# hrnr/map-merge

Hardware: NVIDIA B200
Metric: pairwise_registrations_per_sec (higher is better)
Workload: dtype f32

## Files before the change

map-merge_b200/csrc/exact_math.h:

```cpp
#pragma once
#include <math.h>
#include <stdint.h>
#include <string.h>

#if defined(__CUDACC__)
#define MM_HD __host__ __device__ __forceinline__
#else
#define MM_HD inline
#endif

namespace mm3d {
namespace em {

MM_HD double bits_to_double(uint64_t u)
{
  double d;
  memcpy(&d, &u, sizeof(d));
  return d;
}

MM_HD float bits_to_float(uint32_t u)
{
  float f;
  memcpy(&f, &u, sizeof(f));
  return f;
}

MM_HD float expf_(float x)
{
  if (x != x) return x;
  if (x < -104.0f) return 0.0f;
  if (x > 88.72f) return INFINITY;
  const float n = rintf(x * 1.44269504088896341f);
  float r = x - n * 0.693359375f;
  r = r - n * -2.12194440e-4f;
  float p = 1.9875691500e-4f;
  p = p * r + 1.3981999507e-3f;
  p = p * r + 8.3334519073e-3f;
  p = p * r + 4.1665795894e-2f;
  p = p * r + 1.6666665459e-1f;
  p = p * r + 5.0000001201e-1f;
  const float y = (p * (r * r) + r) + 1.0f;
  int ni = (int)n;
  const int h = ni / 2;
  const float s1 = bits_to_float((uint32_t)(127 + h) << 23);
  const float s2 = bits_to_float((uint32_t)(127 + (ni - h)) << 23);
  return (y * s1) * s2;
}

MM_HD float atanf_pos_(float x, float* lo)
{
  float y0, y0lo;
  if (x > 2.414213562373095f) {
    y0 = 1.57079637050628662109375f;
    y0lo = -4.37113900018624283e-8f;
    x = -(1.0f / x);
  } else if (x > 0.4142135623730950f) {
    y0 = 0.785398185253143310546875f;
    y0lo = -2.18556950009312142e-8f;
    x = (x - 1.0f) / (x + 1.0f);
  } else {
    y0 = 0.0f;
    y0lo = 0.0f;
  }
  const float z = x * x;
  float p = 8.05374449538e-2f;
  p = p * z - 1.38776856032e-1f;
  p = p * z + 1.99777106478e-1f;
  p = p * z - 3.33329491539e-1f;
  const float corr = p * z * x + y0lo;
  const float hi = y0 + x;
  *lo = ((y0 - hi) + x) + corr;
  return hi;
}

MM_HD float atan2f_(float y, float x)
{
  if (x != x || y != y) return x + y;
  const float ax = fabsf(x), ay = fabsf(y);
  float hi = 0.0f, lo = 0.0f;
  if (!(ax == 0.0f && ay == 0.0f)) hi = atanf_pos_(ay / ax, &lo);
  float a;
  if (signbit(x)) {
    const float d = 3.1415927410125732421875f - hi;
    a = d + (-8.74227800037248566e-8f - lo);
  } else {
    a = hi + lo;
  }
  return signbit(y) ? -a : a;
}

MM_HD double cos_small_(double t)
{
  const double t2 = t * t;
  double s = 1.0 / 6402373705728000.0;
  s = 1.0 / 20922789888000.0 - t2 * s;
  s = 1.0 / 87178291200.0 - t2 * s;
  s = 1.0 / 479001600.0 - t2 * s;
  s = 1.0 / 3628800.0 - t2 * s;
  s = 1.0 / 40320.0 - t2 * s;
  s = 1.0 / 720.0 - t2 * s;
  s = 1.0 / 24.0 - t2 * s;
  s = 0.5 - t2 * s;
  return 1.0 - t2 * s;
}

MM_HD double sin_small_(double t)
{
  const double t2 = t * t;
  double s = 1.0 / 121645100408832000.0;
  s = 1.0 / 355687428096000.0 - t2 * s;
  s = 1.0 / 1307674368000.0 - t2 * s;
  s = 1.0 / 6227020800.0 - t2 * s;
  s = 1.0 / 39916800.0 - t2 * s;
  s = 1.0 / 362880.0 - t2 * s;
  s = 1.0 / 5040.0 - t2 * s;
  s = 1.0 / 120.0 - t2 * s;
  s = 1.0 / 6.0 - t2 * s;
  return t * (1.0 - t2 * s);
}

MM_HD float cosf_small_(float t) { return (float)cos_small_((double)t); }
MM_HD float sinf_small_(float t) { return (float)sin_small_((double)t); }

template <typename T>
MM_HD T sqrt_(T v);
template <>
MM_HD float sqrt_<float>(float v) { return sqrtf(v); }
template <>
MM_HD double sqrt_<double>(double v) { return sqrt(v); }

template <typename T>
MM_HD T det3(const T* m)
{
  return m[0] * (m[4] * m[8] - m[5] * m[7]) - m[1] * (m[3] * m[8] - m[5] * m[6]) +
         m[2] * (m[3] * m[7] - m[4] * m[6]);
}

template <typename T>
MM_HD void svd3(const T* A, T* U, T* s, T* V)
{
  T a[9];
  for (int i = 0; i < 9; ++i) {
    a[i] = A[i];
    V[i] = T(0);
  }
  V[0] = V[4] = V[8] = T(1);
  const T eps = sizeof(T) == 4 ? T(1.1920929e-7) : T(2.220446049250313e-16);
  for (int sweep = 0; sweep < 30; ++sweep) {
    bool rotated = false;
    for (int p = 0; p < 2; ++p) {
      for (int q = p + 1; q < 3; ++q) {
        T alpha = T(0), beta = T(0), gamma = T(0);
        for (int i = 0; i < 3; ++i) {
          alpha += a[i * 3 + p] * a[i * 3 + p];
          beta += a[i * 3 + q] * a[i * 3 + q];
          gamma += a[i * 3 + p] * a[i * 3 + q];
        }
        if (gamma == T(0)) continue;
        if (fabs(gamma) <= eps * sqrt_<T>(alpha * beta)) continue;
        rotated = true;
        const T zeta = (beta - alpha) / (T(2) * gamma);
        const T t = (zeta >= T(0) ? T(1) : T(-1)) / (fabs(zeta) + sqrt_<T>(T(1) + zeta * zeta));
        const T c = T(1) / sqrt_<T>(T(1) + t * t);
        const T sn = c * t;
        for (int i = 0; i < 3; ++i) {
          const T ap = a[i * 3 + p], aq = a[i * 3 + q];
          a[i * 3 + p] = c * ap - sn * aq;
          a[i * 3 + q] = sn * ap + c * aq;
          const T vp = V[i * 3 + p], vq = V[i * 3 + q];
          V[i * 3 + p] = c * vp - sn * vq;
          V[i * 3 + q] = sn * vp + c * vq;
        }
      }
    }
    if (!rotated) break;
  }
  T n[3];
  for (int j = 0; j < 3; ++j)
    n[j] = sqrt_<T>(a[j] * a[j] + a[3 + j] * a[3 + j] + a[6 + j] * a[6 + j]);
  int ord[3] = {0, 1, 2};
  for (int i = 0; i < 2; ++i)
    for (int j = i + 1; j < 3; ++j)
      if (n[ord[j]] > n[ord[i]]) {
        int tmp = ord[i];
        ord[i] = ord[j];
        ord[j] = tmp;
      }
  T Vs[9], As[9];
  for (int j = 0; j < 3; ++j) {
    s[j] = n[ord[j]];
    for (int i = 0; i < 3; ++i) {
      Vs[i * 3 + j] = V[i * 3 + ord[j]];
      As[i * 3 + j] = a[i * 3 + ord[j]];
    }
  }
  for (int i = 0; i < 9; ++i) V[i] = Vs[i];
  const T tiny = s[0] * eps * T(8);
  int rank = 0;
  for (int j = 0; j < 3; ++j)
// ... 154 lines not shown
  const float* v;
  float l;
  if (l1 >= l2 && l1 >= l3) {
    v = v1;
    l = l1;
  } else if (l2 >= l1 && l2 >= l3) {
    v = v2;
    l = l2;
  } else {
    v = v3;
    l = l3;
  }
  const float inv = sqrtf(l);
  vec[0] = v[0] / inv;
  vec[1] = v[1] / inv;
  vec[2] = v[2] / inv;
}

MM_HD void eig3_sym_d(const double* a_in, double* val, double* vec)
{
  double a[9];
  for (int i = 0; i < 9; ++i) {
    a[i] = a_in[i];
    vec[i] = 0.0;
  }
  vec[0] = vec[4] = vec[8] = 1.0;
  for (int sweep = 0; sweep < 50; ++sweep) {
    const double off = a[1] * a[1] + a[2] * a[2] + a[5] * a[5];
    const double diag = a[0] * a[0] + a[4] * a[4] + a[8] * a[8];
    if (off <= 1e-32 * diag || off == 0.0) break;
    for (int p = 0; p < 2; ++p)
      for (int q = p + 1; q < 3; ++q) {
        const double apq = a[p * 3 + q];
        if (apq == 0.0) continue;
        const double theta = (a[q * 3 + q] - a[p * 3 + p]) / (2.0 * apq);
        const double t = (theta >= 0.0 ? 1.0 : -1.0) / (fabs(theta) + sqrt(theta * theta + 1.0));
        const double c = 1.0 / sqrt(t * t + 1.0), sn = t * c;
        for (int k = 0; k < 3; ++k) {
          const double akp = a[k * 3 + p], akq = a[k * 3 + q];
          a[k * 3 + p] = c * akp - sn * akq;
          a[k * 3 + q] = sn * akp + c * akq;
        }
        for (int k = 0; k < 3; ++k) {
          const double apk = a[p * 3 + k], aqk = a[q * 3 + k];
          a[p * 3 + k] = c * apk - sn * aqk;
          a[q * 3 + k] = sn * apk + c * aqk;
        }
        for (int k = 0; k < 3; ++k) {
          const double vkp = vec[k * 3 + p], vkq = vec[k * 3 + q];
          vec[k * 3 + p] = c * vkp - sn * vkq;
          vec[k * 3 + q] = sn * vkp + c * vkq;
        }
      }
  }
  val[0] = a[0];
  val[1] = a[4];
  val[2] = a[8];
  for (int i = 0; i < 2; ++i)
    for (int j = i + 1; j < 3; ++j)
      if (val[j] < val[i]) {
        const double tv = val[i];
        val[i] = val[j];
        val[j] = tv;
        for (int k = 0; k < 3; ++k) {
          const double tt = vec[k * 3 + i];
          vec[k * 3 + i] = vec[k * 3 + j];
          vec[k * 3 + j] = tt;
        }
      }
}

MM_HD double atan01_d_(double z)
{
  z = z / (1.0 + sqrt(1.0 + z * z));
  z = z / (1.0 + sqrt(1.0 + z * z));
  const double z2 = z * z;
  double s = 1.0 / 23.0;
  s = 1.0 / 21.0 - z2 * s;
  s = 1.0 / 19.0 - z2 * s;
  s = 1.0 / 17.0 - z2 * s;
  s = 1.0 / 15.0 - z2 * s;
  s = 1.0 / 13.0 - z2 * s;
  s = 1.0 / 11.0 - z2 * s;
  s = 1.0 / 9.0 - z2 * s;
  s = 1.0 / 7.0 - z2 * s;
  s = 1.0 / 5.0 - z2 * s;
  s = 1.0 / 3.0 - z2 * s;
  s = 1.0 - z2 * s;
  return 4.0 * (z * s);
}
MM_HD double atan2_d_(double y, double x)
{
  const double kPi = 3.14159265358979323846;
  if (x != x || y != y) return x + y;
  const double ax = fabs(x), ay = fabs(y);
  double a;
  if (ax == 0.0 && ay == 0.0) a = 0.0;
  else if (ay <= ax) a = atan01_d_(ay / ax);
  else a = 0.5 * kPi - atan01_d_(ax / ay);
  if (signbit(x)) a = kPi - a;
  return signbit(y) ? -a : a;
}
MM_HD double acos_d_(double c)
{
  return atan2_d_(sqrt((1.0 - c) * (1.0 + c)), c);
}

MM_HD float dist2_3(float ax, float ay, float az, float bx, float by, float bz)
{
  const float dx = ax - bx, dy = ay - by, dz = az - bz;
  float r = dx * dx;
  r += dy * dy;
  r += dz * dz;
  return r;
}

MM_HD void transform_point(const float* m, float x, float y, float z, float* ox, float* oy, float* oz)
{
  *ox = ((m[0] * x + m[1] * y) + m[2] * z) + m[3];
  *oy = ((m[4] * x + m[5] * y) + m[6] * z) + m[7];
  *oz = ((m[8] * x + m[9] * y) + m[10] * z) + m[11];
}

#define MM3D_FIX1_SCALE 4294967296.0
#define MM3D_FIX2_SCALE 16777216.0
#define MM3D_FIXD_SCALE 68719476736.0
MM_HD long long to_fix(double v, double scale)
{
#if defined(__CUDA_ARCH__)
  return __double2ll_rn(v * scale);
#else
  return (long long)rint(v * scale);
#endif
}

MM_HD long long to_fix32_pos(float v)
{
  unsigned int b;
#if defined(__CUDA_ARCH__)
  b = __float_as_uint(v);
#else
  memcpy(&b, &v, 4);
#endif
  const int e = (int)((b >> 23) & 0xffu);
  const unsigned long long m = (unsigned long long)(b & 0x7fffffu) | (e ? 0x800000ull : 0ull);
  const int sh = (e ? e : 1) - 118;
  if (sh >= 0) return (long long)(m << sh);
  const int s = -sh;
  if (s > 25) return 0;
  const unsigned long long r = m >> s, rem = m & ((1ull << s) - 1ull), half = 1ull << (s - 1);
  return (long long)(r + ((rem > half || (rem == half && (r & 1ull))) ? 1ull : 0ull));
}

}
}
```

map-merge_b200/csrc/features.cu:

```cuda
#include <algorithm>
#include <cmath>
#include <limits>

#include "mm3d_internal.cuh"
#include "pair_features.cuh"

namespace mm3d {

namespace {

constexpr int FB = 128;

static int radius_voxels(double radius, float leaf) { return (int)std::ceil(radius / (double)leaf) + 1; }

static int max_n(const std::vector<CloudView>& in)
{
  int mx = 0;
  for (const CloudView& v : in) mx = std::max(mx, v.n);
  return mx;
}

static std::vector<Seg> make_segs(const std::vector<int>& ns, int* total)
{
  std::vector<Seg> segs(ns.size());
  int off = 0;
  for (size_t m = 0; m < ns.size(); ++m) {
    segs[m].off = off;
    segs[m].n = ns[m];
    off += ns[m];
  }
  *total = off;
  return segs;
}

struct OutlierJob {
  GridView g;
  uint32_t* flags;
  int* counts;
};

__global__ void __launch_bounds__(FB) outlier_kernel(const OutlierJob* __restrict__ jobs, float r2, int rv, int min_nb)
{
  const OutlierJob& j = jobs[blockIdx.y];
  const int k = blockIdx.x * blockDim.x + threadIdx.x;
  if (k >= j.g.n) return;
  const float4 q = j.g.pts[k];
  int cnt = 0;
  for_each_in_radius(j.g, true, q.x, q.y, q.z, r2, rv, [&](int, const float4&, float) { ++cnt; });
  const int oi = j.g.orig ? j.g.orig[k] : k;
  j.flags[oi] = cnt > min_nb ? 1u : 0u;
  if (j.counts) j.counts[oi] = cnt;
}

struct CompactJob {
  const float4* src;
  const uint32_t* flags;
  const uint32_t* pos;
  float4* dst;
  int n;
};
__global__ void __launch_bounds__(256) compact_points_kernel(const CompactJob* __restrict__ jobs)
{
  const CompactJob& j = jobs[blockIdx.y];
  const int i = blockIdx.x * blockDim.x + threadIdx.x;
  if (i >= j.n) return;
  if (j.flags[i]) j.dst[j.pos[i]] = j.src[i];
}

struct NormalJob {
  GridView g;
  float4* normals;
};

__global__ void __launch_bounds__(FB) normals_kernel(const NormalJob* __restrict__ jobs, float r2, int rv)
{
  const NormalJob& j = jobs[blockIdx.y];
  const int k = blockIdx.x * blockDim.x + threadIdx.x;
  const bool live = k < j.g.n;
  const float4 q = live ? j.g.pts[k] : make_float4(0.f, 0.f, 0.f, 0.f);
  float a0 = 0.f, a1 = 0.f, a2 = 0.f, a3 = 0.f, a4 = 0.f, a5 = 0.f, a6 = 0.f, a7 = 0.f, a8 = 0.f;
  int cnt = 0;
  for_each_in_radius(j.g, live, q.x, q.y, q.z, r2, rv, [&](int, const float4& p, float) {
    a0 += p.x * p.x; a1 += p.x * p.y; a2 += p.x * p.z;
    a3 += p.y * p.y; a4 += p.y * p.z; a5 += p.z * p.z;
    a6 += p.x; a7 += p.y; a8 += p.z;
    ++cnt;
  });
  if (!live) return;
  const int oi = j.g.orig ? j.g.orig[k] : k;
  if (cnt < 3) {
    const float nanv = __int_as_float(0x7fc00000);
    j.normals[oi] = make_float4(nanv, nanv, nanv, nanv);
    return;
  }
  const float n = (float)cnt;
  a0 /= n; a1 /= n; a2 /= n; a3 /= n; a4 /= n; a5 /= n; a6 /= n; a7 /= n; a8 /= n;
  float cov[9];
  cov[0] = a0 - a6 * a6;
  cov[1] = a1 - a6 * a7;
  cov[2] = a2 - a6 * a8;
  cov[4] = a3 - a7 * a7;
  cov[5] = a4 - a7 * a8;
  cov[8] = a5 - a8 * a8;
  cov[3] = cov[1]; cov[6] = cov[2]; cov[7] = cov[5];
  float ev, vec[3];
  em::eigen33_smallest(cov, &ev, vec);
  float nx = vec[0], ny = vec[1], nz = vec[2];
  const float eig_sum = cov[0] + cov[4] + cov[8];
  const float curv = (eig_sum != 0.f) ? fabsf(ev / eig_sum) : 0.f;
  const float vx = 0.0f - q.x, vy = 0.0f - q.y, vz = 0.0f - q.z;
  const float cos_theta = (vx * nx + vy * ny + vz * nz);
  if (cos_theta < 0.f) { nx *= -1.f; ny *= -1.f; nz *= -1.f; }
  j.normals[oi] = make_float4(nx, ny, nz, curv);
}

struct SiftJob {
  GridView g;
  float* dog;
  uint32_t* flags;
};
struct SiftScales {
  float sigma_sqr[6];
};

__device__ __forceinline__ float sift_intensity(float w)
{
  const uint32_t c = __float_as_uint(w);
  const int r = (c >> 16) & 0xff, g = (c >> 8) & 0xff, b = c & 0xff;
  return (float)(299 * r + 587 * g + 114 * b) / 1000.0f;
}

struct SiftPrepJob {
  const float4* src;
  float4* dst;
  int n;
};
__global__ void __launch_bounds__(256) sift_prep_kernel(const SiftPrepJob* __restrict__ jobs)
{
  const SiftPrepJob& j = jobs[blockIdx.y];
  const int i = blockIdx.x * blockDim.x + threadIdx.x;
  if (i >= j.n) return;
  const float4 p = j.src[i];
  j.dst[i] = make_float4(p.x, p.y, p.z, sift_intensity(p.w));
}

__global__ void __launch_bounds__(FB) sift_scale_space_kernel(const SiftJob* __restrict__ jobs, SiftScales sc, float r2, int rv)
{
  __shared__ long long acc[FB / 32][12][32];
  const SiftJob& j = jobs[blockIdx.y];
  const int lane = threadIdx.x & 31, w = threadIdx.x >> 5;
  const int k = blockIdx.x * (FB / 32) + w;
  if (k >= j.g.n) return;
  const unsigned full = 0xffffffffu;
  const float4 q = j.g.pts[k];
#pragma unroll
  for (int s = 0; s < 12; ++s) acc[w][s][lane] = 0;
  warp_radius_unordered(j.g, q.x, q.y, q.z, r2, rv, [&](bool valid, int, const float4& p, float d2) {
    int cnt = 0;
    if (valid) {
#pragma unroll
      for (int s = 0; s < 6; ++s) cnt += (d2 <= 9 * sc.sigma_sqr[s]) ? 1 : 0;
    }
    int incl = cnt;
#pragma unroll
    for (int o = 1; o < 32; o <<= 1) {
      const int t = __shfl_up_sync(full, incl, o);
      if (lane >= o) incl += t;
    }
    const int total = __shfl_sync(full, incl, 31);
    const int excl = incl - cnt;
    for (int t0 = 0; t0 < total; t0 += 32) {
      const int t = t0 + lane;
      int L = 0;
#pragma unroll
      for (int step = 16; step >= 1; step >>= 1) {
        const int v = __shfl_sync(full, incl, L + step - 1);
        if (v <= t) L += step;
      }
      L = min(L, 31);
      const float od2 = __shfl_sync(full, d2, L), oval = __shfl_sync(full, p.w, L);
      const int oex = __shfl_sync(full, excl, L), ocnt = __shfl_sync(full, cnt, L);
      if (t < total) {
        const int s = (6 - ocnt) + (t - oex);
        const float wgt = em::expf_(-0.5f * od2 / sc.sigma_sqr[s]);
        acc[w][s][lane] += em::to_fix32_pos(oval * wgt);
        acc[w][6 + s][lane] += em::to_fix32_pos(wgt);
      }
    }
  });
  long long mine = 0;
  if (lane < 12)
    for (int l = 0; l < 32; ++l) mine += acc[w][lane][(l + lane) & 31];
  const long long den = __shfl_down_sync(full, mine, 6);
  float resp = 0.f;
  if (lane < 6) resp = (float)((double)mine / MM3D_FIX1_SCALE) / (float)((double)den / MM3D_FIX1_SCALE);
  const float prev = __shfl_up_sync(full, resp, 1);
  if (lane >= 1 && lane < 6) j.dog[(size_t)k * 5 + (lane - 1)] = resp - prev;
}

constexpr int EX_CAP = 384;

__global__ void __launch_bounds__(FB) sift_extrema_kernel(const SiftJob* __restrict__ jobs, float min_contrast)
{
  __shared__ int queues[FB / 32][64];
  __shared__ float cd[FB / 32][EX_CAP];
  __shared__ int ci[FB / 32][EX_CAP];
  const SiftJob& j = jobs[blockIdx.y];
  const int w = threadIdx.x >> 5, lane = threadIdx.x & 31;
  const int k = blockIdx.x * (FB / 32) + w;
  if (k >= j.g.n) return;
  const float4 q = j.g.pts[k];
  constexpr int K = 25;
  const int rv_max = max(max(j.g.div_v[0], j.g.div_v[1]), j.g.div_v[2]) + 2;
  int m = 0;
  bool overflow = false;
  for (int rv = 3;; rv = rv + max(1, rv / 3)) {
    const float rad = (float)rv * j.g.leaf;
    int fill = 0;
    m = warp_radius_query(j.g, q.x, q.y, q.z, rad * rad, rv + 1, queues[w], [&](int slot) {
      const int at = fill + lane;
      if (at < EX_CAP) {
        const float4 p = j.g.pts[slot];
        cd[w][at] = em::dist2_3(q.x, q.y, q.z, p.x, p.y, p.z);
        ci[w][at] = slot;
      }
      fill += 32;
    });
    __syncwarp();
    if (m > EX_CAP) { overflow = true; break; }
    if (m >= K || rv > rv_max) break;
  }
  float mn[5], mx[5];
#pragma unroll
  for (int s = 0; s < 5; ++s) { mn[s] = 3.402823466e+38f; mx[s] = -3.402823466e+38f; }
  if (!overflow) {
    for (int c = lane; c < m; c += 32) {
      const float d = cd[w][c];
      const int id = ci[w][c];
      int rank = 0;
      for (int o = 0; o < m; ++o) {
        const float od = cd[w][o];
        rank += (od < d || (od == d && ci[w][o] < id)) ? 1 : 0;
      }
      if (rank < K) {
        const float* dg = j.dog + (size_t)id * 5;
#pragma unroll
        for (int s = 0; s < 5; ++s) {
          const float v = dg[s];
          mn[s] = fminf(mn[s], v);
          mx[s] = fmaxf(mx[s], v);
        }
      }
    }
  } else if (lane == 0) {
    float bd[K];
    int bi[K];
    int cnt = 0, rv = 3;
    for (;;) {
      cnt = 0;
      const float rad = (float)rv * j.g.leaf;
      for_each_in_radius(j.g, true, q.x, q.y, q.z, rad * rad, rv + 1, [&](int idx, const float4&, float d2) {
        if (cnt == K && !(d2 < bd[K - 1] || (d2 == bd[K - 1] && idx < bi[K - 1]))) return;
        int pos = (cnt < K) ? cnt : K - 1;
        while (pos > 0 && (d2 < bd[pos - 1] || (d2 == bd[pos - 1] && idx < bi[pos - 1]))) {
          bd[pos] = bd[pos - 1];
          bi[pos] = bi[pos - 1];
          --pos;
        }
        bd[pos] = d2;
        bi[pos] = idx;
        if (cnt < K) ++cnt;
      });
      if (cnt == K || rv > rv_max) break;
      rv *= 2;
    }
    for (int t = 0; t < cnt; ++t) {
      const float* dg = j.dog + (size_t)bi[t] * 5;
#pragma unroll
      for (int s = 0; s < 5; ++s) {
        mn[s] = fminf(mn[s], dg[s]);
        mx[s] = fmaxf(mx[s], dg[s]);
      }
    }
  }
#pragma unroll
  for (int s = 0; s < 5; ++s) {
#pragma unroll
    for (int o = 16; o > 0; o >>= 1) {
      mn[s] = fminf(mn[s], __shfl_xor_sync(0xffffffffu, mn[s], o));
      mx[s] = fmaxf(mx[s], __shfl_xor_sync(0xffffffffu, mx[s], o));
    }
  }
  if (lane == 0) {
#pragma unroll
    for (int s = 1; s < 4; ++s) {
      const float val = j.dog[(size_t)k * 5 + s];
      uint32_t f = 0;
      if (fabsf(val) >= min_contrast) {
        if ((val == mn[s]) && (val < mn[s - 1]) && (val < mn[s + 1])) f = 1;
        else if ((val == mx[s]) && (val > mx[s - 1]) && (val > mx[s + 1])) f = 1;
      }
      j.flags[(size_t)k * 3 + (s - 1)] = f;
    }
  }
}

struct SiftEmitJob {
  const float4* pts;
  const uint32_t* flags;
  const uint32_t* pos;
  float4* dst;
  int n3;
};
__global__ void __launch_bounds__(256) sift_emit_kernel(const SiftEmitJob* __restrict__ jobs)
{
  const SiftEmitJob& j = jobs[blockIdx.y];
  const int i = blockIdx.x * blockDim.x + threadIdx.x;
  if (i >= j.n3) return;
  if (!j.flags[i]) return;
  const float4 p = j.pts[i / 3];
  j.dst[j.pos[i]] = make_float4(p.x, p.y, p.z, __uint_as_float(0xff000000u));
}

struct FpfhJob {
  GridView g;
  const float4* normals;
  const float4* kp;
  int nk;
  uint32_t* need;
  float* spfh;
  float* desc_raw;
  uint32_t* valid3;
};

__global__ void __launch_bounds__(FB) fpfh_mark_kernel(const FpfhJob* __restrict__ jobs, float r2, int rv)
{
  const FpfhJob& j = jobs[blockIdx.y];
  const int t = blockIdx.x * (FB / 32) + (threadIdx.x >> 5);
  if (t >= j.nk) return;
  const float4 q = j.kp[t];
  warp_radius_unordered(j.g, q.x, q.y, q.z, r2, rv, [&](bool valid, int k, const float4&, float) {
    if (valid) j.need[k] = 1u;
  });
}

__global__ void __launch_bounds__(FB) spfh_kernel(const FpfhJob* __restrict__ jobs, float r2, int rv, BinTable bins)
{
  __shared__ int queues[FB / 32][64];
  __shared__ unsigned short cnt[FB / 32][33][32];
  __shared__ float thr[3][12];
  if (threadIdx.x < 36) (&thr[0][0])[threadIdx.x] = (&bins.t[0][0])[threadIdx.x];
  const int w = threadIdx.x >> 5, lane = threadIdx.x & 31;
  for (int b = 0; b < 33; ++b) cnt[w][b][lane] = 0;
  __syncthreads();
  const FpfhJob& j = jobs[blockIdx.y];
  const int k = blockIdx.x * (FB / 32) + w;
  if (k >= j.g.n || !j.need[k]) return;
  const float4 p = j.g.pts[k];
  const float4 np = j.normals[j.g.orig ? j.g.orig[k] : k];
  const int n = warp_radius_query(j.g, p.x, p.y, p.z, r2, rv, queues[w], [&](int q) {
    if (q == k) return;
    const float4 pq = j.g.pts[q];
    const float4 nq = j.normals[j.g.orig ? j.g.orig[q] : q];
    float f1, f2, f3;
    if (!pair_features(p, np, pq, nq, &f1, &f2, &f3)) return;
    const int h1 = lookup_bin(thr[0], 11, f1, 11.0f * 0.15915494f, 3.14159274f);
    const int h2 = lookup_bin(thr[1], 11, f2, 5.5f, 1.0f);
    const int h3 = lookup_bin(thr[2], 11, f3, 5.5f, 1.0f);
    cnt[w][h1][lane]++;
    cnt[w][11 + h2][lane]++;
    cnt[w][22 + h3][lane]++;
  });
  __syncwarp();
  const float hist_incr = 100.0f / (float)(n - 1);
  float* out = j.spfh + (size_t)k * 33;
  for (int b = lane; b < 33; b += 32) {
    unsigned int c = 0;
    for (int l = 0; l < 32; ++l) c += cnt[w][b][(l + lane) & 31];
    float h = 0.f;
    for (unsigned int t = 0; t < c; ++t) h += hist_incr;
    out[b] = h;
  }
}

__global__ void __launch_bounds__(FB) fpfh_weight_kernel(const FpfhJob* __restrict__ jobs, float r2, int rv)
{
  __shared__ int queues[FB / 32][64];
  const FpfhJob& j = jobs[blockIdx.y];
  const int w = threadIdx.x >> 5, lane = threadIdx.x & 31;
  const int kp = blockIdx.x * (FB / 32) + w;
  if (kp >= j.nk) return;
  const unsigned full = 0xffffffffu;
  const float4 q = j.kp[kp];
  const int f = lane < 11 ? 0 : (lane < 22 ? 1 : 2);
  const int base = f * 11;
  float acc = 0.f, acc32 = 0.f;
  double sum = 0.0;
  const int found = warp_radius_query<true>(j.g, q.x, q.y, q.z, r2, rv, queues[w], [&](int slot) {
    float weight = 0.f;
    if (slot >= 0) {
      const float4 p = j.g.pts[slot];
      const float d2 = em::dist2_3(q.x, q.y, q.z, p.x, p.y, p.z);
      weight = d2 == 0.f ? 0.f : 1.0f / d2;
    }
    const unsigned have = __ballot_sync(full, slot >= 0);
    const int m = __popc(have);
    for (int t = 0; t < m; ++t) {
      const int s = __shfl_sync(full, slot, t);
      const float wt = __shfl_sync(full, weight, t);
      if (wt == 0.f) continue;
      const float* h = j.spfh + (size_t)s * 33;
      const float val = h[lane] * wt;
      const float val32 = lane == 0 ? h[32] * wt : 0.f;
      acc += val;
      acc32 += val32;
      const float v32 = __shfl_sync(full, val32, 0);
#pragma unroll
      for (int i = 0; i < 11; ++i) {
        float v = __shfl_sync(full, val, (base + i) & 31);
        if (base + i == 32) v = v32;
        sum += (double)v;
      }
    }
  });
  if (sum != 0.0) sum = 100.0 / sum;
  const float scale = (float)__shfl_sync(full, sum, base);
  const float scale2 = (float)__shfl_sync(full, sum, 22);
  const float v = acc * scale;
  const float v32 = acc32 * scale2;
  bool fin = isfinite(v);
  if (lane == 0) fin = fin && isfinite(v32);
  const bool ok = __all_sync(full, fin) && found > 0;
  j.desc_raw[(size_t)kp * 33 + lane] = v;
  if (lane == 0) j.desc_raw[(size_t)kp * 33 + 32] = v32;
  if (lane < 3) j.valid3[kp * 3 + lane] = ok ? 1u : 0u;
}
// ... 179 lines not shown
  if (total == 0) return;
  const double rd = (double)radius_f;
  const float r2 = (float)(rd * rd);
  const int rv = radius_voxels(rd, idx[0].v.leaf);
  DBuf<uint32_t> flags(c, total), pos(c, total);
  std::vector<DBuf<float>> resp(M);
  std::vector<HarrisJob> jobs(M);
  for (int m = 0; m < M; ++m) {
    resp[m].alloc(c, ns[m]);
    jobs[m].g = idx[m].v;
    jobs[m].normals = normals[m];
    jobs[m].response = resp[m].p;
    jobs[m].flags = flags.p + segs[m].off;
    jobs[m].cloud = clouds[m].pts;
    jobs[m].corners = nullptr;
    jobs[m].n_corners = 0;
  }
  DBuf<HarrisJob> dj = to_device(c, jobs);
  const dim3 grid((mx + FB - 1) / FB, M);
  { double b = 0; for (int m = 0; m < M; ++m) b += 36.0 * ns[m]; MM_BYTES(c, b); }
  MM_LAUNCH(c, harris_response_kernel, grid, FB, 0, dj.p, r2, rv);
  { double b = 0; for (int m = 0; m < M; ++m) b += 24.0 * ns[m]; MM_BYTES(c, b); }
  MM_LAUNCH(c, harris_nms_kernel, grid, FB, 0, dj.p, r2, rv, threshold);
  std::vector<int> totals;
  scan_flags_batch(c, flags.p, pos.p, segs, totals);
  std::vector<HarrisEmitJob> ej(M);
  int mxc = 0;
  for (int m = 0; m < M; ++m) {
    keypoints[m].n = totals[m];
    keypoints[m].pts.alloc(c, totals[m]);
    ej[m] = HarrisEmitJob{clouds[m].pts, flags.p + segs[m].off, pos.p + segs[m].off, keypoints[m].pts.p, ns[m]};
    jobs[m].corners = keypoints[m].pts.p;
    jobs[m].n_corners = totals[m];
    mxc = std::max(mxc, totals[m]);
  }
  DBuf<HarrisEmitJob> dej = to_device(c, ej);
  MM_LAUNCH(c, harris_emit_kernel, dim3((mx + 255) / 256, M), 256, 0, dej.p);
  if (unrefined_dbg)
    for (int m = 0; m < M; ++m) {
      (*unrefined_dbg)[m].n = totals[m];
      (*unrefined_dbg)[m].pts.alloc(c, totals[m]);
      if (totals[m]) MM_CUDA(cudaMemcpyAsync((*unrefined_dbg)[m].pts.p, keypoints[m].pts.p, (size_t)totals[m] * sizeof(float4), cudaMemcpyDeviceToDevice, c.stream));
    }
  if (mxc > 0) {
    DBuf<HarrisJob> dj2 = to_device(c, jobs);
    MM_LAUNCH(c, harris_refine_kernel, dim3((mxc + FB - 1) / FB, M), FB, 0, dj2.p, r2, rv);
  }
  if (response_dbg)
    for (int m = 0; m < M; ++m) (*response_dbg)[m] = std::move(resp[m]);
}

void remove_outliers_batch(Ctx& c, const std::vector<CloudView>& clouds, const std::vector<DIndex>& idx, double radius, int min_nb,
                           std::vector<DCloud>& out, std::vector<DBuf<int>>* counts)
{
  const int M = (int)clouds.size();
  out.clear();
  out.resize(M);
  if (counts) { counts->clear(); counts->resize(M); }
  if (M == 0) return;
  std::vector<int> ns(M);
  for (int m = 0; m < M; ++m) ns[m] = clouds[m].n;
  int total = 0;
  std::vector<Seg> segs = make_segs(ns, &total);
  if (total == 0) return;
  DBuf<uint32_t> flags(c, total), pos(c, total);
  std::vector<OutlierJob> jobs(M);
  for (int m = 0; m < M; ++m) {
    jobs[m].g = idx[m].v;
    jobs[m].flags = flags.p + segs[m].off;
    jobs[m].counts = nullptr;
    if (counts) {
      (*counts)[m].alloc(c, ns[m]);
      jobs[m].counts = (*counts)[m].p;
    }
  }
  DBuf<OutlierJob> dj = to_device(c, jobs);
  const float r2 = (float)(radius * radius);
  const int rv = radius_voxels(radius, idx[0].v.leaf);
  const int mx = max_n(clouds);
  { double b = 0; for (int m = 0; m < M; ++m) b += 20.0 * ns[m]; MM_BYTES(c, b); }
  MM_LAUNCH(c, outlier_kernel, dim3((mx + FB - 1) / FB, M), FB, 0, dj.p, r2, rv, min_nb);
  std::vector<int> totals;
  scan_flags_batch(c, flags.p, pos.p, segs, totals);
  std::vector<CompactJob> cj(M);
  for (int m = 0; m < M; ++m) {
    out[m].n = totals[m];
    out[m].pts.alloc(c, totals[m]);
    cj[m] = CompactJob{clouds[m].pts, flags.p + segs[m].off, pos.p + segs[m].off, out[m].pts.p, ns[m]};
  }
  DBuf<CompactJob> dcj = to_device(c, cj);
  MM_LAUNCH(c, compact_points_kernel, dim3((mx + 255) / 256, M), 256, 0, dcj.p);
}

void normals_batch(Ctx& c, const std::vector<CloudView>& clouds, const std::vector<DIndex>& idx, double radius,
                   std::vector<DBuf<float4>>& normals)
{
  const int M = (int)clouds.size();
  normals.clear();
  normals.resize(M);
  if (M == 0) return;
  std::vector<NormalJob> jobs(M);
  for (int m = 0; m < M; ++m) {
    normals[m].alloc(c, clouds[m].n);
    jobs[m].g = idx[m].v;
    jobs[m].normals = normals[m].p;
  }
  const int mx = max_n(clouds);
  if (mx == 0) return;
  DBuf<NormalJob> dj = to_device(c, jobs);
  const float r2 = (float)(radius * radius);
  const int rv = radius_voxels(radius, idx[0].v.leaf);
  { double b = 0; for (int m = 0; m < M; ++m) b += 32.0 * clouds[m].n; MM_BYTES(c, b); }
  MM_LAUNCH(c, normals_kernel, dim3((mx + FB - 1) / FB, M), FB, 0, dj.p, r2, rv);
}

void sift_batch(Ctx& c, const std::vector<CloudView>& clouds, float min_scale, int n_octaves, int n_scales, float min_contrast,
                std::vector<DCloud>& keypoints, std::vector<DBuf<float>>* dog0)
{
  const int M = (int)clouds.size();
  keypoints.clear();
  keypoints.resize(M);
  if (dog0) { dog0->clear(); dog0->resize(M); }
  if (M == 0) return;
  if (n_scales != 3) throw std::runtime_error("sift_batch: the reference path uses 3 scales per octave");
  std::vector<char> active(M, 1);
  std::vector<CloudView> cur = clouds;
  std::vector<std::vector<DCloud>> octave_kp(M);
  std::vector<std::vector<DCloud>> keep_alive;
  float scale = min_scale;
  for (int oct = 0; oct < n_octaves; ++oct) {
    const float s = 1.0f * scale;
    std::vector<CloudView> in(M);
    for (int m = 0; m < M; ++m) in[m] = active[m] ? cur[m] : CloudView{nullptr, 0};
    keep_alive.emplace_back();
    std::vector<DCloud>& oc = keep_alive.back();
    std::vector<VoxGeom> ogeom;
    voxel_downsample_batch(c, in, s, oc, &ogeom);
    bool any = false;
    std::vector<CloudView> ov(M);
    for (int m = 0; m < M; ++m) {
      if (active[m] && oc[m].n < 25) active[m] = 0;
      ov[m] = active[m] ? oc[m].view() : CloudView{nullptr, 0};
      cur[m] = oc[m].view();
      any = any || active[m];
    }
    if (!any) break;
    std::vector<DIndex> idx;
    build_index_batch(c, ov, s, 2, 0, 0, idx, nullptr, &ogeom);
    float scales[6];
    SiftScales sc;
    for (int i = 0; i < 6; ++i) {
      scales[i] = scale * powf(2.0f, (1.0f * (float)i - 1.0f) / (float)n_scales);
      sc.sigma_sqr[i] = powf(scales[i], 2.0f);
    }
    const float max_radius = 3.0f * scales[5];
    const float r2 = (float)((double)max_radius * (double)max_radius);
    const int rv = radius_voxels((double)max_radius, s);
    std::vector<int> ns(M), n3(M);
    for (int m = 0; m < M; ++m) { ns[m] = ov[m].n; n3[m] = ov[m].n * 3; }
    int total3 = 0;
    std::vector<Seg> segs3 = make_segs(n3, &total3);
    DBuf<uint32_t> flags(c, total3), pos(c, total3);
    std::vector<DBuf<float>> dog(M);
    std::vector<SiftJob> jobs(M);
    for (int m = 0; m < M; ++m) {
      dog[m].alloc(c, (size_t)ns[m] * 5);
      jobs[m].g = idx[m].v;
      jobs[m].dog = dog[m].p;
      jobs[m].flags = flags.p + segs3[m].off;
    }
    DBuf<SiftJob> dj = to_device(c, jobs);
    const int mx = max_n(ov);
    const dim3 grid((mx + FB - 1) / FB, M);
    std::vector<DBuf<float4>> pi(M);
    std::vector<SiftPrepJob> pj(M);
    std::vector<SiftJob> jobs_ss = jobs;
    for (int m = 0; m < M; ++m) {
      if (idx[m].v.orig) throw std::runtime_error("sift_batch: octave cloud is not in voxel order");
      pi[m].alloc(c, ns[m]);
      pj[m] = SiftPrepJob{ov[m].pts, pi[m].p, ns[m]};
      jobs_ss[m].g.pts = pi[m].p;
    }
    DBuf<SiftPrepJob> dpj = to_device(c, pj);
    MM_LAUNCH(c, sift_prep_kernel, dim3((mx + 255) / 256, M), 256, 0, dpj.p);
    DBuf<SiftJob> djs = to_device(c, jobs_ss);
    { double b = 0; for (int m = 0; m < M; ++m) b += 36.0 * ns[m]; MM_BYTES(c, b); }
    MM_LAUNCH(c, sift_scale_space_kernel, dim3((mx + FB / 32 - 1) / (FB / 32), M), FB, 0, djs.p, sc, r2, rv);
    { double b = 0; for (int m = 0; m < M; ++m) b += 48.0 * ns[m]; MM_BYTES(c, b); }
    MM_LAUNCH(c, sift_extrema_kernel, dim3((mx + FB / 32 - 1) / (FB / 32), M), FB, 0, dj.p, min_contrast);
    std::vector<int> totals;
    scan_flags_batch(c, flags.p, pos.p, segs3, totals);
    std::vector<SiftEmitJob> ej(M);
    for (int m = 0; m < M; ++m) {
      octave_kp[m].emplace_back();
      DCloud& k = octave_kp[m].back();
      k.n = totals[m];
      k.pts.alloc(c, totals[m]);
      ej[m] = SiftEmitJob{ov[m].pts, flags.p + segs3[m].off, pos.p + segs3[m].off, k.pts.p, n3[m]};
    }
    DBuf<SiftEmitJob> dej = to_device(c, ej);
    MM_LAUNCH(c, sift_emit_kernel, dim3((mx * 3 + 255) / 256, M), 256, 0, dej.p);
    if (dog0 && oct == 0)
      for (int m = 0; m < M; ++m) (*dog0)[m] = std::move(dog[m]);
    scale *= 2;
  }
  for (int m = 0; m < M; ++m) {
    int tot = 0;
    for (const DCloud& k : octave_kp[m]) tot += k.n;
    keypoints[m].n = tot;
    keypoints[m].pts.alloc(c, tot);
    int off = 0;
    for (const DCloud& k : octave_kp[m]) {
      if (k.n) MM_CUDA(cudaMemcpyAsync(keypoints[m].pts.p + off, k.pts.p, (size_t)k.n * sizeof(float4), cudaMemcpyDeviceToDevice, c.stream));
      off += k.n;
    }
  }
}

void fpfh_batch(Ctx& c, const std::vector<CloudView>& clouds, const std::vector<DIndex>& idx, const std::vector<const float4*>& normals,
                std::vector<DCloud>& keypoints, double radius, std::vector<DBuf<float>>& desc, std::vector<DBuf<float>>* spfh_dbg)
{
  const int M = (int)clouds.size();
  desc.clear();
  desc.resize(M);
  if (spfh_dbg) { spfh_dbg->clear(); spfh_dbg->resize(M); }
  if (M == 0) return;
  std::vector<int> nks(M);
  int mxk = 0;
  for (int m = 0; m < M; ++m) { nks[m] = keypoints[m].n; mxk = std::max(mxk, nks[m]); }
  int totalk = 0;
  std::vector<Seg> segk = make_segs(nks, &totalk);
  const int mx = max_n(clouds);
  if (totalk == 0 || mx == 0) {
    for (int m = 0; m < M; ++m) { keypoints[m].n = 0; keypoints[m].pts.release(); }
    return;
  }
  std::vector<DBuf<uint32_t>> need(M), valid3(M);
  std::vector<DBuf<float>> spfh(M), raw(M);
  std::vector<FpfhJob> jobs(M);
  for (int m = 0; m < M; ++m) {
    need[m].alloc(c, clouds[m].n);
    need[m].zero(c);
    spfh[m].alloc(c, (size_t)clouds[m].n * 33);
    if (spfh_dbg) spfh[m].zero(c);
    raw[m].alloc(c, (size_t)nks[m] * 33);
    valid3[m].alloc(c, (size_t)nks[m] * 3);
    jobs[m].g = idx[m].v;
    jobs[m].normals = normals[m];
    jobs[m].kp = keypoints[m].pts.p;
    jobs[m].nk = nks[m];
    jobs[m].need = need[m].p;
    jobs[m].spfh = spfh[m].p;
    jobs[m].desc_raw = raw[m].p;
    jobs[m].valid3 = valid3[m].p;
  }
  DBuf<FpfhJob> dj = to_device(c, jobs);
  const float r2 = (float)(radius * radius);
  const int rv = radius_voxels(radius, idx[0].v.leaf);
  MM_LAUNCH(c, fpfh_mark_kernel, dim3((mxk + FB / 32 - 1) / (FB / 32), M), FB, 0, dj.p, r2, rv);
  { double b = 0; for (int m = 0; m < M; ++m) b += (32.0 + 132.0 + 4.0) * clouds[m].n; MM_BYTES(c, b); }
  static const BinTable bins = make_bin_table(11);
  MM_LAUNCH(c, spfh_kernel, dim3((mx + FB / 32 - 1) / (FB / 32), M), FB, 0, dj.p, r2, rv, bins);
  { double b = 0; for (int m = 0; m < M; ++m) b += (16.0 + 132.0) * clouds[m].n + (16.0 + 132.0) * nks[m]; MM_BYTES(c, b); }
  MM_LAUNCH(c, fpfh_weight_kernel, dim3((mxk + FB / 32 - 1) / (FB / 32), M), FB, 0, dj.p, r2, rv);
  DBuf<uint32_t> flags(c, totalk), pos(c, totalk);
  std::vector<FpfhFlagJob> fj(M);
  for (int m = 0; m < M; ++m) fj[m] = FpfhFlagJob{valid3[m].p, flags.p + segk[m].off, nks[m]};
  DBuf<FpfhFlagJob> dfj = to_device(c, fj);
  MM_LAUNCH(c, fpfh_flag_kernel, dim3((mxk + 255) / 256, M), 256, 0, dfj.p);
  std::vector<int> totals;
  scan_flags_batch(c, flags.p, pos.p, segk, totals);
  std::vector<DCloud> kept(M);
  std::vector<FpfhEmitJob> ej(M);
  for (int m = 0; m < M; ++m) {
    kept[m].n = totals[m];
    kept[m].pts.alloc(c, totals[m]);
    desc[m].alloc(c, (size_t)totals[m] * 33);
    ej[m] = FpfhEmitJob{keypoints[m].pts.p, raw[m].p, flags.p + segk[m].off, pos.p + segk[m].off, kept[m].pts.p, desc[m].p, nks[m]};
  }
  DBuf<FpfhEmitJob> dej = to_device(c, ej);
  MM_LAUNCH(c, fpfh_emit_kernel, dim3((mxk * 33 + 255) / 256, M), 256, 0, dej.p);
  for (int m = 0; m < M; ++m) keypoints[m] = std::move(kept[m]);
  if (spfh_dbg)
    for (int m = 0; m < M; ++m) (*spfh_dbg)[m] = std::move(spfh[m]);
}

}
```

Measured before the change: 1063.

## Fuse SIFT K-nearest search into scale-space pass and speed up weight math

The scale-space kernel now records neighbour candidates in three distance bands while it already walks the radius query. It ranks them into a per-point 25-nearest list, and the extrema kernel reuses that list instead of redoing the expanding radius search; it falls back to the old search when the bands overflow. The per-candidate work distribution replaces the shuffle prefix scan and binary search with ballots plus a shared owner table. Division is done through a precomputed reciprocal with two FMA refinement steps, and fixed-point conversion uses __float2ll_rn. This adds shared memory, a global nn buffer and extra writes, with a risk of rounding differences in the exact-math path.

```diff
diff --git a/map-merge_b200/csrc/exact_math.h b/map-merge_b200/csrc/exact_math.h
--- a/map-merge_b200/csrc/exact_math.h
+++ b/map-merge_b200/csrc/exact_math.h
@@ -26,11 +26,8 @@
   return f;
 }
 
-MM_HD float expf_(float x)
-{
-  if (x != x) return x;
-  if (x < -104.0f) return 0.0f;
-  if (x > 88.72f) return INFINITY;
+MM_HD float expf_core_(float x)
+{
   const float n = rintf(x * 1.44269504088896341f);
   float r = x - n * 0.693359375f;
   r = r - n * -2.12194440e-4f;
@@ -46,6 +43,14 @@
   const float s1 = bits_to_float((uint32_t)(127 + h) << 23);
   const float s2 = bits_to_float((uint32_t)(127 + (ni - h)) << 23);
   return (y * s1) * s2;
+}
+
+MM_HD float expf_(float x)
+{
+  if (x != x) return x;
+  if (x < -104.0f) return 0.0f;
+  if (x > 88.72f) return INFINITY;
+  return expf_core_(x);
 }
 
 MM_HD float atanf_pos_(float x, float* lo)
@@ -506,5 +511,16 @@
   return (long long)(r + ((rem > half || (rem == half && (r & 1ull))) ? 1ull : 0ull));
 }
 
-}
-}
+#if defined(__CUDACC__)
+__device__ __forceinline__ long long to_fix32_pos_dev(float v) { return __float2ll_rn(v * 4294967296.0f); }
+
+__device__ __forceinline__ float div_rn_recip(float a, float b, float y)
+{
+  const float q0 = a * y;
+  const float q1 = __fmaf_rn(__fmaf_rn(-q0, b, a), y, q0);
+  return __fmaf_rn(__fmaf_rn(-q1, b, a), y, q1);
+}
+#endif
+
+}
+}
diff --git a/map-merge_b200/csrc/features.cu b/map-merge_b200/csrc/features.cu
--- a/map-merge_b200/csrc/features.cu
+++ b/map-merge_b200/csrc/features.cu
@@ -114,13 +114,19 @@
   j.normals[oi] = make_float4(nx, ny, nz, curv);
 }
 
+constexpr int SIFT_K = 25;
+
 struct SiftJob {
   GridView g;
   float* dog;
   uint32_t* flags;
+  int* nn;
 };
 struct SiftScales {
   float sigma_sqr[6];
+  float mant[6];
+  float inv_mant[6];
+  float neg_half_pow2[6];
 };
 
 __device__ __forceinline__ float sift_intensity(float w)
@@ -144,85 +150,142 @@
   j.dst[i] = make_float4(p.x, p.y, p.z, sift_intensity(p.w));
 }
 
-__global__ void __launch_bounds__(FB) sift_scale_space_kernel(const SiftJob* __restrict__ jobs, SiftScales sc, float r2, int rv)
-{
-  __shared__ long long acc[FB / 32][12][32];
+template <typename F>
+__device__ __forceinline__ void sift_rank_nearest(const float* cd, const int* ci, int m, int kk, F found)
+{
+  const int lane = threadIdx.x & 31;
+  for (int c = lane; c < m; c += 32) {
+    const float d = cd[c];
+    const int id = ci[c];
+    int rank = 0;
+    for (int o = 0; o < m; ++o) {
+      const float od = cd[o];
+      rank += (od < d || (od == d && ci[o] < id)) ? 1 : 0;
+    }
+    if (rank < kk) found(rank, id);
+  }
+}
+
+constexpr int NN_CAP = 96;
+
+__global__ void __launch_bounds__(FB, 8) sift_scale_space_kernel(const SiftJob* __restrict__ jobs, SiftScales sc, float r2, int rv)
+{
+  __shared__ longlong2 acc[FB / 32][6][32];
+  __shared__ float2 cand[FB / 32][32];
+  __shared__ unsigned char owner[FB / 32][192];
+  __shared__ float nd[FB / 32][3][NN_CAP];
+  __shared__ int ni[FB / 32][3][NN_CAP];
+  __shared__ float4 div_tab[6];
+  if (threadIdx.x == 0)
+#pragma unroll
+    for (int s = 0; s < 6; ++s) div_tab[s] = make_float4(sc.mant[s], sc.inv_mant[s], sc.neg_half_pow2[s], 0.f);
+  __syncthreads();
   const SiftJob& j = jobs[blockIdx.y];
   const int lane = threadIdx.x & 31, w = threadIdx.x >> 5;
   const int k = blockIdx.x * (FB / 32) + w;
   if (k >= j.g.n) return;
-  const unsigned full = 0xffffffffu;
+  const unsigned full = 0xffffffffu, below = (1u << lane) - 1u;
   const float4 q = j.g.pts[k];
 #pragma unroll
-  for (int s = 0; s < 12; ++s) acc[w][s][lane] = 0;
-  warp_radius_unordered(j.g, q.x, q.y, q.z, r2, rv, [&](bool valid, int, const float4& p, float d2) {
+  for (int s = 0; s < 6; ++s) acc[w][s][lane] = make_longlong2(0, 0);
+  int n_band[3] = {0, 0, 0};
+  warp_radius_unordered(j.g, q.x, q.y, q.z, r2, rv, [&](bool valid, int idx, const float4& p, float d2) {
     int cnt = 0;
     if (valid) {
 #pragma unroll
       for (int s = 0; s < 6; ++s) cnt += (d2 <= 9 * sc.sigma_sqr[s]) ? 1 : 0;
     }
-    int incl = cnt;
-#pragma unroll
-    for (int o = 1; o < 32; o <<= 1) {
-      const int t = __shfl_up_sync(full, incl, o);
-      if (lane >= o) incl += t;
-    }
-    const int total = __shfl_sync(full, incl, 31);
-    const int excl = incl - cnt;
-    for (int t0 = 0; t0 < total; t0 += 32) {
-      const int t = t0 + lane;
-      int L = 0;
-#pragma unroll
-      for (int step = 16; step >= 1; step >>= 1) {
-        const int v = __shfl_sync(full, incl, L + step - 1);
-        if (v <= t) L += step;
+#pragma unroll
+    for (int b = 0; b < 3; ++b) {
+      const unsigned in = __ballot_sync(full, cnt == 6 - b);
+      const int at = n_band[b] + __popc(in & below);
+      if (cnt == 6 - b && at < NN_CAP) {
+        nd[w][b][at] = d2;
+        ni[w][b][at] = idx;
       }
-      L = min(L, 31);
-      const float od2 = __shfl_sync(full, d2, L), oval = __shfl_sync(full, p.w, L);
-      const int oex = __shfl_sync(full, excl, L), ocnt = __shfl_sync(full, cnt, L);
-      if (t < total) {
-        const int s = (6 - ocnt) + (t - oex);
-        const float wgt = em::expf_(-0.5f * od2 / sc.sigma_sqr[s]);
-        acc[w][s][lane] += em::to_fix32_pos(oval * wgt);
-        acc[w][6 + s][lane] += em::to_fix32_pos(wgt);
-      }
-    }
+      n_band[b] += __popc(in);
+    }
+    const unsigned b0 = __ballot_sync(full, cnt & 1), b1 = __ballot_sync(full, cnt & 2), b2 = __ballot_sync(full, cnt & 4);
+    const int total = __popc(b0) + 2 * __popc(b1) + 4 * __popc(b2);
+    if (total == 0) return;
+    const int excl = __popc(b0 & below) + 2 * __popc(b1 & below) + 4 * __popc(b2 & below);
+    if (cnt) cand[w][lane] = make_float2(d2, p.w);
+#pragma unroll
+    for (int i = 0; i < 6; ++i)
+      if (i < cnt) owner[w][excl + i] = (unsigned char)(lane | ((6 - cnt + i) << 5));
+    __syncwarp();
+    for (int t = lane; t < total; t += 32) {
+      const int o = owner[w][t], s = o >> 5;
+      const float2 c = cand[w][o & 31];
+      const float4 dv = div_tab[s];
+      const float x = em::div_rn_recip(c.x * dv.z, dv.x, dv.y);
+      const float wgt = em::expf_core_(x);
+      longlong2 a = acc[w][s][lane];
+      a.x += em::to_fix32_pos_dev(c.y * wgt);
+      a.y += em::to_fix32_pos_dev(wgt);
+      acc[w][s][lane] = a;
+    }
+    __syncwarp();
   });
-  long long mine = 0;
-  if (lane < 12)
-    for (int l = 0; l < 32; ++l) mine += acc[w][lane][(l + lane) & 31];
-  const long long den = __shfl_down_sync(full, mine, 6);
+  long long num = 0, den = 0;
+  if (lane < 6)
+    for (int l = 0; l < 32; ++l) {
+      const longlong2 a = acc[w][lane][(l + lane) & 31];
+      num += a.x;
+      den += a.y;
+    }
   float resp = 0.f;
-  if (lane < 6) resp = (float)((double)mine / MM3D_FIX1_SCALE) / (float)((double)den / MM3D_FIX1_SCALE);
+  if (lane < 6) resp = (float)((double)num / MM3D_FIX1_SCALE) / (float)((double)den / MM3D_FIX1_SCALE);
   const float prev = __shfl_up_sync(full, resp, 1);
   if (lane >= 1 && lane < 6) j.dog[(size_t)k * 5 + (lane - 1)] = resp - prev;
+  int* nn = j.nn + (size_t)k * SIFT_K;
+  int base = 0, cut = 0;
+  bool known = false;
+#pragma unroll
+  for (int b = 0; b < 3; ++b) {
+    if (known || n_band[b] > NN_CAP) break;
+    if (base + n_band[b] >= SIFT_K) {
+      known = true;
+      cut = b;
+    } else {
+      base += n_band[b];
+    }
+  }
+  if (!known) {
+    if (lane == 0) nn[0] = -1;
+    return;
+  }
+  __syncwarp();
+  int at = 0;
+#pragma unroll
+  for (int b = 0; b < 2; ++b)
+    if (b < cut) {
+      for (int c = lane; c < n_band[b]; c += 32) nn[at + c] = ni[w][b][c];
+      at += n_band[b];
+    }
+  const int n_cut = cut == 0 ? n_band[0] : (cut == 1 ? n_band[1] : n_band[2]);
+  sift_rank_nearest(nd[w][cut], ni[w][cut], n_cut, SIFT_K - base, [&](int rank, int id) { nn[base + rank] = id; });
 }
 
 constexpr int EX_CAP = 384;
 
-__global__ void __launch_bounds__(FB) sift_extrema_kernel(const SiftJob* __restrict__ jobs, float min_contrast)
-{
-  __shared__ int queues[FB / 32][64];
-  __shared__ float cd[FB / 32][EX_CAP];
-  __shared__ int ci[FB / 32][EX_CAP];
-  const SiftJob& j = jobs[blockIdx.y];
-  const int w = threadIdx.x >> 5, lane = threadIdx.x & 31;
-  const int k = blockIdx.x * (FB / 32) + w;
-  if (k >= j.g.n) return;
+__device__ __forceinline__ void sift_extrema_search(const SiftJob& j, int k, float* cd, int* ci, int* queue, float (&mn)[5], float (&mx)[5])
+{
+  const int lane = threadIdx.x & 31;
   const float4 q = j.g.pts[k];
-  constexpr int K = 25;
+  constexpr int K = SIFT_K;
   const int rv_max = max(max(j.g.div_v[0], j.g.div_v[1]), j.g.div_v[2]) + 2;
   int m = 0;
   bool overflow = false;
   for (int rv = 3;; rv = rv + max(1, rv / 3)) {
     const float rad = (float)rv * j.g.leaf;
     int fill = 0;
-    m = warp_radius_query(j.g, q.x, q.y, q.z, rad * rad, rv + 1, queues[w], [&](int slot) {
+    m = warp_radius_query(j.g, q.x, q.y, q.z, rad * rad, rv + 1, queue, [&](int slot) {
       const int at = fill + lane;
       if (at < EX_CAP) {
         const float4 p = j.g.pts[slot];
-        cd[w][at] = em::dist2_3(q.x, q.y, q.z, p.x, p.y, p.z);
-        ci[w][at] = slot;
+        cd[at] = em::dist2_3(q.x, q.y, q.z, p.x, p.y, p.z);
+        ci[at] = slot;
       }
       fill += 32;
     });
@@ -230,28 +293,16 @@
     if (m > EX_CAP) { overflow = true; break; }
     if (m >= K || rv > rv_max) break;
   }
-  float mn[5], mx[5];
-#pragma unroll
-  for (int s = 0; s < 5; ++s) { mn[s] = 3.402823466e+38f; mx[s] = -3.402823466e+38f; }
   if (!overflow) {
-    for (int c = lane; c < m; c += 32) {
-      const float d = cd[w][c];
-      const int id = ci[w][c];
-      int rank = 0;
-      for (int o = 0; o < m; ++o) {
-        const float od = cd[w][o];
-        rank += (od < d || (od == d && ci[w][o] < id)) ? 1 : 0;
+    sift_rank_nearest(cd, ci, m, K, [&](int, int id) {
+      const float* dg = j.dog + (size_t)id * 5;
+#pragma unroll
+      for (int s = 0; s < 5; ++s) {
+        const float v = dg[s];
+        mn[s] = fminf(mn[s], v);
+        mx[s] = fmaxf(mx[s], v);
       }
-      if (rank < K) {
-        const float* dg = j.dog + (size_t)id * 5;
-#pragma unroll
-        for (int s = 0; s < 5; ++s) {
-          const float v = dg[s];
-          mn[s] = fminf(mn[s], v);
-          mx[s] = fmaxf(mx[s], v);
-        }
-      }
-    }
+    });
   } else if (lane == 0) {
     float bd[K];
     int bi[K];
@@ -282,6 +333,34 @@
         mx[s] = fmaxf(mx[s], dg[s]);
       }
     }
+  }
+}
+
+__global__ void __launch_bounds__(FB) sift_extrema_kernel(const SiftJob* __restrict__ jobs, float min_contrast)
+{
+  __shared__ int queues[FB / 32][64];
+  __shared__ float cd[FB / 32][EX_CAP];
+  __shared__ int ci[FB / 32][EX_CAP];
+  const SiftJob& j = jobs[blockIdx.y];
+  const int w = threadIdx.x >> 5, lane = threadIdx.x & 31;
+  const int k = blockIdx.x * (FB / 32) + w;
+  if (k >= j.g.n) return;
+  float mn[5], mx[5];
+#pragma unroll
+  for (int s = 0; s < 5; ++s) { mn[s] = 3.402823466e+38f; mx[s] = -3.402823466e+38f; }
+  const int nb = lane < SIFT_K ? j.nn[(size_t)k * SIFT_K + lane] : 0;
+  if (__shfl_sync(0xffffffffu, nb, 0) >= 0) {
+    if (lane < SIFT_K) {
+      const float* dg = j.dog + (size_t)nb * 5;
+#pragma unroll
+      for (int s = 0; s < 5; ++s) {
+        const float v = dg[s];
+        mn[s] = fminf(mn[s], v);
+        mx[s] = fmaxf(mx[s], v);
+      }
+    }
+  } else {
+    sift_extrema_search(j, k, cd[w], ci[w], queues[w], mn, mx);
   }
 #pragma unroll
   for (int s = 0; s < 5; ++s) {
@@ -767,6 +846,10 @@
     for (int i = 0; i < 6; ++i) {
       scales[i] = scale * powf(2.0f, (1.0f * (float)i - 1.0f) / (float)n_scales);
       sc.sigma_sqr[i] = powf(scales[i], 2.0f);
+      int e = 0;
+      sc.mant[i] = 2.0f * std::frexp(sc.sigma_sqr[i], &e);
+      sc.inv_mant[i] = 1.0f / sc.mant[i];
+      sc.neg_half_pow2[i] = std::ldexp(-0.5f, 1 - e);
     }
     const float max_radius = 3.0f * scales[5];
     const float r2 = (float)((double)max_radius * (double)max_radius);
@@ -777,12 +860,15 @@
     std::vector<Seg> segs3 = make_segs(n3, &total3);
     DBuf<uint32_t> flags(c, total3), pos(c, total3);
     std::vector<DBuf<float>> dog(M);
+    std::vector<DBuf<int>> nn(M);
     std::vector<SiftJob> jobs(M);
     for (int m = 0; m < M; ++m) {
       dog[m].alloc(c, (size_t)ns[m] * 5);
+      nn[m].alloc(c, (size_t)ns[m] * SIFT_K);
       jobs[m].g = idx[m].v;
       jobs[m].dog = dog[m].p;
       jobs[m].flags = flags.p + segs3[m].off;
+      jobs[m].nn = nn[m].p;
     }
     DBuf<SiftJob> dj = to_device(c, jobs);
     const int mx = max_n(ov);
@@ -799,10 +885,11 @@
     DBuf<SiftPrepJob> dpj = to_device(c, pj);
     MM_LAUNCH(c, sift_prep_kernel, dim3((mx + 255) / 256, M), 256, 0, dpj.p);
     DBuf<SiftJob> djs = to_device(c, jobs_ss);
-    { double b = 0; for (int m = 0; m < M; ++m) b += 36.0 * ns[m]; MM_BYTES(c, b); }
-    MM_LAUNCH(c, sift_scale_space_kernel, dim3((mx + FB / 32 - 1) / (FB / 32), M), FB, 0, djs.p, sc, r2, rv);
-    { double b = 0; for (int m = 0; m < M; ++m) b += 48.0 * ns[m]; MM_BYTES(c, b); }
-    MM_LAUNCH(c, sift_extrema_kernel, dim3((mx + FB / 32 - 1) / (FB / 32), M), FB, 0, dj.p, min_contrast);
+    const dim3 wgrid((mx + FB / 32 - 1) / (FB / 32), M);
+    { double b = 0; for (int m = 0; m < M; ++m) b += (36.0 + 4.0 * SIFT_K) * ns[m]; MM_BYTES(c, b); }
+    MM_LAUNCH(c, sift_scale_space_kernel, wgrid, FB, 0, djs.p, sc, r2, rv);
+    { double b = 0; for (int m = 0; m < M; ++m) b += (48.0 + 4.0 * SIFT_K) * ns[m]; MM_BYTES(c, b); }
+    MM_LAUNCH(c, sift_extrema_kernel, wgrid, FB, 0, dj.p, min_contrast);
     std::vector<int> totals;
     scan_flags_batch(c, flags.p, pos.p, segs3, totals);
     std::vector<SiftEmitJob> ej(M);
```

New measurement: 1109, median of 6. +4.3%, better.
